# talmolab/VNL-Brax-Imitation

Hardware: AMD Instinct MI355X
Metric: env-steps/sec (whole node), rodent imitation, num_envs=4096/GPU (higher is better)
Workload: dtype f32; 1 GPU; rodent imitation rollout, single groom clip, 4096 envs/GPU: intention-policy forward (HIP) -> RodentTracking.step (5 substeps, CG 6/6) -> auto-reset on -> Transition logging (unroll 20, the 20 steps replayed as one captured hipGraph); envs_per_gpu=4096, clips=1, parallelism=env-sharded x1, no data-path collective

## Files before the change

__graft_entry__.py:

```python
from __future__ import annotations

import os
import sys

ROOT = os.path.dirname(os.path.abspath(__file__))
if ROOT not in sys.path:
    sys.path.insert(0, ROOT)


def build() -> None:
    import vnl_brax_imitation_amd
    from vnl_brax_imitation_amd.csrc import build as hip_build

    from concurrent.futures import ThreadPoolExecutor

    with ThreadPoolExecutor(8) as pool:
        futs = {v: pool.submit(hip_build.build, variant=v)
                for v in ("product", "spill", "noblk", "nospec", "tail", "plain", "vmemplain", "ldsplain")}
        paths = {v: f.result() for v, f in futs.items()}
    path = paths["product"]
    assert all(os.path.exists(p_) for p_ in paths.values()), paths
    from oracle import oracle as _oracle

    _oracle.build()
    from vnl_brax_imitation_amd import _lib

    _lib.load_library(path)
    print(f"[build] {path} ok; oracle ok")


def smoke() -> None:
    import numpy as np
    import torch

    sys.path.insert(0, os.path.join(ROOT, "tests"))
    import helpers as H
    from vnl_brax_imitation_amd.envs.rodent import RodentTracking

    assert torch.cuda.is_available(), "smoke() needs a HIP device"
    B = 256
    env = RodentTracking(H.reference_clip(), num_envs=B, device="cuda:0", **H.env_kwargs())
    rng = np.random.default_rng(0)
    sf = rng.integers(0, 235, B).astype(np.int32)
    noise = (1e-3 * rng.standard_normal((B, 74))).astype(np.float32)
    st = env.reset(start_frame=torch.from_numpy(sf), noise=torch.from_numpy(noise))
    act = np.clip(0.3 * rng.standard_normal((B, 30)), -1, 1).astype(np.float32)
    o = H.make_oracle(env, "f64")
    ost = o.env_reset(sf, noise)
    e_reset = H.scaled_err(st.pipeline_state.qacc_warmstart.cpu().numpy(), ost["qacc_warmstart"])
    e_obs = H.scaled_err(st.obs.cpu().numpy(), ost["obs"])
    import parity as P

    o32 = H.make_oracle(env, "f32")
    st, err, dev, rep, ost = P.control_step_follow(env, o, o32, sf, noise, act)
    torch.cuda.synchronize()
    print(f"[smoke] reset qacc err {e_reset:.2e}, obs err {e_obs:.2e}; control step vs oracle (following the product's "
          f"solver decisions): qvel err max {err['qvel'].max():.2e} median {np.median(err['qvel']):.2e}, qpos max "
          f"{err['qpos'].max():.2e}; reward {st.reward.mean().item():.5f} vs {ost['reward'].mean():.5f}")
    w = int(np.argmax(err["qvel"]))
    print(f"[smoke] worst env {w}: product vs float64 oracle {err['qvel'][w]:.2e}, float32 oracle vs float64 oracle "
          f"{dev['qvel'][w]:.2e} on the same env (bound: max(1e-5, {P.K_SENS} x that))")
    cp, co = P.compliance(err), P.compliance(dev)
    print(f"[smoke] envs within 1e-5 after ONE CONTROL STEP ({B} envs): product qpos {cp['qpos']:.3f} qvel {cp['qvel']:.3f} | "
          f"float32 oracle qpos {co['qpos']:.3f} qvel {co['qvel']:.3f}")
    env1 = RodentTracking(H.reference_clip(), num_envs=B, device="cuda:0", **{**H.env_kwargs(), "n_frames": 1})
    o1, o1_32 = H.make_oracle(env1, "f64"), H.make_oracle(env1, "f32")
    _, err1, dev1, rep1, _ = P.control_step_follow(env1, o1, o1_32, sf, noise, act)
    cp1, co1 = P.compliance(err1), P.compliance(dev1)
    print(f"[smoke] envs within 1e-5 after ONE SUBSTEP: product qpos {cp1['qpos']:.3f} qvel {cp1['qvel']:.3f} | float32 oracle "
          f"qpos {co1['qpos']:.3f} qvel {co1['qvel']:.3f}; followed decisions: {P.assert_legitimate(rep1)}")
    for f, idx in P.bound_violations(err1, dev1).items():
        assert len(idx) == 0, (f, idx[:8], err1[f][idx[:8]], dev1[f][idx[:8]])
    assert e_reset < 1e-4 and e_obs < 1e-5, (e_reset, e_obs)
    P.check_control_step(err, dev, rep)
    assert np.abs(st.reward.cpu().numpy() - ost["reward"]).max() < 2e-4
    assert np.array_equal(st.done.cpu().numpy(), ost["done"].astype(np.float32))
    assert torch.isfinite(st.obs).all()


if __name__ == "__main__":
    build()
    if "--smoke" in sys.argv:
        smoke()
```

vnl-brax-imitation_amd/csrc/build.py:

```python
from __future__ import annotations

import os
import subprocess
import sys

HERE = os.path.dirname(os.path.abspath(__file__))
SOURCES = ["vnl_lib.hip", "vnl_policy.hip", "vnl_ppo.hip", "vnl_domain.hip"]
DEPS = SOURCES + ["vnl_env_kernels.h", "vnl_body.h", "vnl_types.h", "vnl_philox.h", "vnl_policy_train.h", "../../include/vnl.h"]
OUT = os.path.join(HERE, "libvnl.so")

VARIANTS = {
    "product": ("libvnl.so", ["-DVNL_KERNEL_ATTR=__attribute__((amdgpu_waves_per_eu(2,2)))"]),
    "prof": ("libvnl_prof.so", ["-DVNL_PROFILE", "-DVNL_KERNEL_ATTR=__attribute__((amdgpu_waves_per_eu(2,2)))"]),
    "knobs": ("libvnl_knobs.so", ["-DVNL_STAGE_KNOBS", "-DVNL_KERNEL_ATTR=__attribute__((amdgpu_waves_per_eu(2,2)))"]),
    "spill": ("libvnl_spill.so", ["-DVNL_KERNEL_ATTR=__attribute__((amdgpu_waves_per_eu(4,4)))"]),
    "noblk": ("libvnl_noblk.so", ["-DVNL_NO_BLK", "-DVNL_KERNEL_ATTR=__attribute__((amdgpu_waves_per_eu(2,2)))"]),
    "tail": ("libvnl_tail.so", ["-DVNL_SOLVER_TAIL", "-DVNL_KERNEL_ATTR=__attribute__((amdgpu_waves_per_eu(2,2)))"]),
    "plain": ("libvnl_plain.so", ["-DVNL_SOLVER_PLAIN", "-DVNL_KERNEL_ATTR=__attribute__((amdgpu_waves_per_eu(2,2)))"]),
    "vmemplain": ("libvnl_vmemplain.so", ["-DVNL_VMEM_PLAIN", "-DVNL_KERNEL_ATTR=__attribute__((amdgpu_waves_per_eu(2,2)))"]),
    "ldsplain": ("libvnl_ldsplain.so", ["-DVNL_LDS_PLAIN", "-DVNL_KERNEL_ATTR=__attribute__((amdgpu_waves_per_eu(2,2)))"]),
    "nospec": ("libvnl_nospec.so", ["-DVNL_NO_SPEC", "-DVNL_KERNEL_ATTR=__attribute__((amdgpu_waves_per_eu(2,2)))"]),
}
ENV_KERNELS = ("vnl_step_kernel", "vnl_reset_kernel", "vnl_reset_done_kernel")


def resource_usage(stderr_text: str) -> dict:
    out, name = {}, None
    for line in stderr_text.splitlines():
        if "Function Name:" in line:
            name = line.split("Function Name:")[1].split()[0]
            out[name] = {}
        elif name and "remark:" in line:
            body = line.split("remark:")[1].split("[-Rpass")[0].strip()
            key, _, val = body.rpartition(":")
            try:
                out[name][key.strip()] = int(val.strip())
            except ValueError:
                pass
    return out


def build(force: bool = False, verbose: bool = False, profile: bool = False, knobs: bool = False,
          variant: str | None = None) -> str:
    variant = variant or ("prof" if profile else ("knobs" if knobs else "product"))
    fname, defs = VARIANTS[variant]
    out = os.path.join(HERE, fname)
    deps = [os.path.join(HERE, d) for d in DEPS] + [os.path.abspath(__file__)]
    newest = max(os.path.getmtime(d) for d in deps)
    if not force and os.path.exists(out) and os.path.getmtime(out) >= newest:
        return out
    hipcc = os.environ.get("HIPCC", "/opt/rocm/bin/hipcc")
    objdir = os.path.join(HERE, "_obj", variant)
    os.makedirs(objdir, exist_ok=True)
    flags = ["-Rpass-analysis=kernel-resource-usage", "--offload-arch=gfx950", "-O3", "-fno-slp-vectorize", "-std=c++17", "-fPIC"] + \
        defs + os.environ.get("VNL_HIPCC_EXTRA", "").split()
    stamp = " ".join(flags)
    headers = [d for d in deps if not d.endswith(".hip")]
    SRC_DEPS = {"vnl_lib.hip": headers, "vnl_policy.hip": [h for h in headers if h.endswith("vnl.h")] + [os.path.join(HERE, "vnl_policy_train.h"), os.path.join(HERE, "vnl_philox.h")],
                "vnl_ppo.hip": [h for h in headers if h.endswith("vnl.h")] + [os.path.join(HERE, "vnl_policy_train.h")]}
    objs, remarks = [], ""
    for src in SOURCES:
        obj = os.path.join(objdir, src + ".o")
        rem = obj + ".remarks.txt"
        srcdeps = [os.path.join(HERE, src)] + [h for h in SRC_DEPS.get(src, headers) if os.path.exists(h)]
        fresh = (not force and os.path.exists(obj) and os.path.exists(rem) and
                 os.path.getmtime(obj) >= max(os.path.getmtime(d) for d in srcdeps) and
                 open(rem).readline().rstrip("\n") == stamp)
        if not fresh:
            cmd = [hipcc] + flags + ["-c", os.path.join(HERE, src), "-o", obj]
            if verbose:
                print(" ".join(cmd), file=sys.stderr)
            r = subprocess.run(cmd, stderr=subprocess.PIPE, text=True)
            if verbose or r.returncode:
                sys.stderr.write(r.stderr)
            if r.returncode:
                raise subprocess.CalledProcessError(r.returncode, cmd)
            with open(rem, "w") as f:
                f.write(stamp + "\n" + r.stderr)
        objs.append(obj)
        remarks += open(rem).read().split("\n", 1)[1]
    cmd = [hipcc, "--offload-arch=gfx950", "-shared", "-fPIC", "-o", out] + objs
    r = subprocess.run(cmd, stderr=subprocess.PIPE, text=True)
    if r.returncode:
        sys.stderr.write(r.stderr)
        raise subprocess.CalledProcessError(r.returncode, cmd)

    class _R:
        stderr = remarks
    r = _R()
    usage = resource_usage(r.stderr)
    seen = {k: [u for n, u in usage.items() if k in n] for k in ENV_KERNELS}
    missing = [k for k, v in seen.items() if not v or "Occupancy [waves/SIMD]" not in v[0]]
    if missing:
        os.remove(out)
        raise RuntimeError(f"no resource-usage remark for {missing}: cannot check the register budget of this build")
    if variant == "product":
        for k, u in ((k, u) for k, v in seen.items() for u in v):
            if u.get("ScratchSize [bytes/lane]", 0) > 64 or u["Occupancy [waves/SIMD]"] < 2:
                if os.environ.get("VNL_ALLOW_SPILL") != "1":
                    os.remove(out)
                    raise RuntimeError(
                        f"{k}: {u.get('VGPRs')} VGPRs, {u.get('ScratchSize [bytes/lane]')} B scratch per lane, "
                        f"{u['Occupancy [waves/SIMD]']} waves/SIMD -- below the two waves per SIMD without spilling that the "
                        "published numbers were measured with.  Results do not depend on spilling (tests/test_gpu_spill.py); "
                        "this gate keeps a performance regression from shipping silently: set VNL_ALLOW_SPILL=1 to build anyway")
                sys.stderr.write(f"[build] WARNING (performance): {k} uses {u.get('VGPRs')} VGPRs, "
                                 f"{u.get('ScratchSize [bytes/lane]')} B scratch per lane, "
                                 f"{u['Occupancy [waves/SIMD]']} waves/SIMD: below the two waves per SIMD without "
                                 "spilling that the published numbers were measured with\n")
    with open(os.path.join(HERE, fname + ".resources.txt"), "w") as f:
        for n, u in usage.items():
            f.write(n + " " + " ".join(f"{a}={b}" for a, b in sorted(u.items())) + "\n")
    return out


if __name__ == "__main__":
    v = next((k for k in VARIANTS if "--" + k in sys.argv), None)
    if "--profile" in sys.argv:
        v = "prof"
    print(build(force="--force" in sys.argv, verbose=True, variant=v))
```

vnl-brax-imitation_amd/csrc/vnl_policy.hip:

```cpp
#include <hip/hip_runtime.h>
#include <math.h>
#include <stdint.h>
#include <stdio.h>

#include "../../include/vnl.h"
#include "vnl_philox.h"
#include "vnl_policy_train.h"

#define PT 16
#define PTHREADS 1024
#define PNT ((int)blockDim.x)
#define LN_EPS 1e-6f

typedef float v4f __attribute__((ext_vector_type(4)));


__device__ __forceinline__ int dense_col_groups(int N) {
  int G = (N + 63) >> 6, Gp = 1;
  while (Gp < G && Gp < PNT / 64) Gp <<= 1;
  return Gp;
}

template <bool VEC>
__device__ __forceinline__ void dense_tile_t(const float* X, int ldx, int K, const float* __restrict__ params, int w_off,
                                             int b_off, int N, float* Y, int ldy, bool relu, float* P, int split,
                                             int w2_off, int b2_off) {
  const float* __restrict__ bias = params + b_off;
  const float* __restrict__ bias2 = params + b2_off;
  const int tid = threadIdx.x, lane = tid & 63, wave = tid >> 6;
  const int j = lane & 15, kq = lane >> 4;
  const int G = (N + 63) >> 6, Gp = dense_col_groups(N), S = (PNT / 64) / Gp;
  const int g0 = wave & (Gp - 1), s = wave / Gp;
  const int N4 = (N + 3) & ~3;
  const int T = (K + 3) >> 2, Ts = (T + S - 1) / S;
  const int t0 = s * Ts, t1 = min(T, t0 + Ts);
  const float* xr = X + j * ldx + kq;
  float bias_r[4];
#pragma unroll
  for (int q = 0; q < 4; q++) {
    const int e = tid + q * PNT;
    const int c = e % N;
    bias_r[q] = e < PT * N ? (c < split ? bias[c] : bias2[c - split]) : 0.f;
  }
  const int ldw = split < N ? split : N;
  for (int g = g0; g < G; g += Gp) {
    const int c0 = g * 64 + 4 * j;
    auto load_b = [&](int step) -> v4f {
      const int k = 4 * step + kq;
      const float* w = params + (c0 < split ? w_off : w2_off - split) + (size_t)((step < t1 && k < K) ? k : 0) * ldw;
      v4f b;
      if (VEC) {
        b = *(const v4f*)(w + (c0 < N ? c0 : 0));
      } else {
#pragma unroll
        for (int t = 0; t < 4; t++) b[t] = w[c0 + t < N ? c0 + t : 0];
      }
      return b;
    };
    v4f acc[4];
#pragma unroll
    for (int t = 0; t < 4; t++) acc[t] = v4f{0.f, 0.f, 0.f, 0.f};
    auto mma4 = [&](const v4f (&b)[4], int t) {
      float a[4];
#pragma unroll
      for (int u = 0; u < 4; u++) {
        const int step = t + u;
        const bool ok = step < t1 && 4 * step + kq < K;
        float v = xr[ok ? 4 * step : 0];
        a[u] = ok ? v : 0.f;
      }
#pragma unroll
      for (int u = 0; u < 4; u++)
#pragma unroll
        for (int tt = 0; tt < 4; tt++) acc[tt] = __builtin_amdgcn_mfma_f32_16x16x4f32(a[u], b[u][tt], acc[tt], 0, 0, 0);
    };
    v4f b0[4], b1[4];
    if (t0 < t1) {
#pragma unroll
      for (int u = 0; u < 4; u++) b0[u] = load_b(t0 + u);
    }
    for (int t = t0; t < t1; t += 8) {
      const bool more1 = t + 4 < t1, more0 = t + 8 < t1;
      if (more1) {
#pragma unroll
        for (int u = 0; u < 4; u++) b1[u] = load_b(t + 4 + u);
      }
      __builtin_amdgcn_sched_barrier(0);
      mma4(b0, t);
      __builtin_amdgcn_sched_barrier(0);
      if (more0) {
#pragma unroll
        for (int u = 0; u < 4; u++) b0[u] = load_b(t + 8 + u);
      }
      __builtin_amdgcn_sched_barrier(0);
      if (more1) mma4(b1, t + 4);
      __builtin_amdgcn_sched_barrier(0);
    }
    if (c0 < N4) {
#pragma unroll
      for (int i = 0; i < 4; i++)
        *(v4f*)(P + (size_t)(s * PT + kq * 4 + i) * N4 + c0) = v4f{acc[0][i], acc[1][i], acc[2][i], acc[3][i]};
    }
  }
  __syncthreads();
  auto finish = [&](int e, float v) {
    const int r = e / N, c = e - r * N;
    for (int ss = 0; ss < S; ss++) v += P[(size_t)(ss * PT + r) * N4 + c];
    Y[r * ldy + c] = relu ? fmaxf(v, 0.f) : v;
  };
#pragma unroll
  for (int q = 0; q < 4; q++) {
    const int e = tid + q * PNT;
    if (e < PT * N) finish(e, bias_r[q]);
  }
  for (int e = tid + 4 * PNT; e < PT * N; e += PNT) finish(e, e % N < split ? bias[e % N] : bias2[e % N - split]);
  __syncthreads();
}

__device__ __forceinline__ void dense_tile(const float* X, int ldx, int K, const float* __restrict__ params, int w_off,
                                           int b_off, int N, float* Y, int ldy, bool relu, float* P, int split = 1 << 30,
                                           int w2_off = 0, int b2_off = 0) {
  const int ldw = split < N ? split : N;
  if ((ldw & 3) == 0 && ((uintptr_t)params & 15) == 0 && (w_off & 3) == 0 && (w2_off & 3) == 0)
    dense_tile_t<true>(X, ldx, K, params, w_off, b_off, N, Y, ldy, relu, P, split, w2_off, b2_off);
  else
    dense_tile_t<false>(X, ldx, K, params, w_off, b_off, N, Y, ldy, relu, P, split, w2_off, b2_off);
}

__device__ __forceinline__ void store_tile(const float* src, int ld, int nrow, int width, float* __restrict__ dst, int e0) {
  for (int i = threadIdx.x; i < nrow * width; i += PNT) {
    const int r = i / width, c = i - r * width;
    dst[(size_t)(e0 + r) * width + c] = src[r * ld + c];
  }
}

template <bool TRAIN>
__device__ __forceinline__ void layer_norm_rows(float* Y, int ldy, int N, const float* __restrict__ g,
                                                const float* __restrict__ be, float* __restrict__ stats = nullptr, int e0 = 0,
                                                int nrow = 0) {
  const int lane = threadIdx.x & 63, wave = threadIdx.x >> 6;
  const int RPW = PT / (PNT / 64);
  float gr[4], br[4];
#pragma unroll
  for (int q = 0; q < 4; q++) {
    const int c = lane + 64 * q;
    gr[q] = c < N ? g[c] : 0.f, br[q] = c < N ? be[c] : 0.f;
  }
  for (int r = wave * RPW; r < wave * RPW + RPW; r++) {
    float* y = Y + r * ldy;
    float s = 0.f, ss = 0.f;
    for (int c = lane; c < N; c += 64) {
      float v = y[c];
      s += v, ss += v * v;
    }
    for (int o = 32; o > 0; o >>= 1) s += __shfl_xor(s, o), ss += __shfl_xor(ss, o);
    float mean = s / (float)N;
    float var = fmaxf(ss / (float)N - mean * mean, 0.f);
    if (TRAIN) {
      float q = 0.f;
      for (int c = lane; c < N; c += 64) {
        const float d = y[c] - mean;
        q += d * d;
      }
      for (int o = 32; o > 0; o >>= 1) q += __shfl_xor(q, o);
      var = q / (float)N;
    }
    float inv = rsqrtf(var + LN_EPS);
    if (TRAIN && lane == 0 && r < nrow) stats[2 * (size_t)(e0 + r)] = mean, stats[2 * (size_t)(e0 + r) + 1] = inv;
#pragma unroll
    for (int q = 0; q < 4; q++) {
      const int c = lane + 64 * q;
      if (c < N) y[c] = (y[c] - mean) * inv * gr[q] + br[q];
    }
    for (int c = lane + 256; c < N; c += 64) y[c] = (y[c] - mean) * inv * g[c] + be[c];
  }
}

__device__ __forceinline__ void load_tile(const float* __restrict__ src, int nrow, int width, float* dst, int ld,
                                          const float* __restrict__ mean, const float* __restrict__ stdv) {
  const int tid = threadIdx.x, n = nrow * width;
  auto put = [&](int i, float v) {
    const int r = i / width, c = i - r * width;
    if (mean) v = (v - mean[c]) / stdv[c];
    dst[r * ld + c] = v;
  };
  int done = 0;
  if (((uintptr_t)src & 15) == 0) {
    const v4f* s4 = (const v4f*)src;
    const int n4 = n >> 2;
    for (int base = 0; base < n4; base += 4 * PNT) {
      v4f v[4];
#pragma unroll
      for (int u = 0; u < 4; u++) {
        const int i = base + u * PNT + tid;
        v[u] = s4[i < n4 ? i : 0];
      }
#pragma unroll
      for (int u = 0; u < 4; u++) {
        const int i = base + u * PNT + tid;
        if (i < n4) {
#pragma unroll
          for (int q = 0; q < 4; q++) put(4 * i + q, v[u][q]);
        }
      }
    }
    done = n4 << 2;
  }
  for (int i = done + tid; i < n; i += PNT) put(i, src[i]);
  for (int i = n + tid; i < PT * width; i += PNT) {
    const int r = i / width, c = i - r * width;
    dst[r * ld + c] = 0.f;
  }
}

#ifdef VNL_PROFILE
__device__ long long g_policy_stamps[32];
#define POL_STAMP(i)                                                               \
  do {                                                                             \
    if (blockIdx.x == 0 && threadIdx.x == 0) g_policy_stamps[i] = wall_clock64(); \
  } while (0)
extern "C" int vnl_policy_profile_stamps(long long* out) {
  return hipMemcpyFromSymbol(out, HIP_SYMBOL(g_policy_stamps), sizeof(long long) * 32) == hipSuccess ? 0 : -1;
}
#else
#define POL_STAMP(i)
#endif

__device__ __forceinline__ float softplusf(float x) { return x > 20.f ? x : log1pf(expf(x)); }

struct PolicyNoiseDev {
  uint32_t key0, key1;
  const int64_t* step_base;
  int64_t step_offset;
  uint32_t env0;
  float *eps_latent_out, *eps_action_out, *rand_action_out;
};


__device__ __forceinline__ void draw_normal_tile(const PolicyNoiseDev& nz, int64_t step, uint32_t stream, int e0, int nrow, int n,
                                                 float* dst, float* __restrict__ rec) {
  const int nb = (n + 3) >> 2;
  const uint32_t c2 = (uint32_t)step, c3 = ((uint32_t)(step >> 32) << 2) | stream;
  for (int i = threadIdx.x; i < nrow * nb; i += PNT) {
    const int r = i / nb, b = i - r * nb;
    uint32_t x[4];
    philox4x32_10((uint32_t)b, nz.env0 + (uint32_t)(e0 + r), c2, c3, nz.key0, nz.key1, x);
    float v[4];
    box_muller(x[0], x[1], v[0], v[1]);
    box_muller(x[2], x[3], v[2], v[3]);
    *(v4f*)(dst + (r * nb + b) * 4) = v4f{v[0], v[1], v[2], v[3]};
    if (rec) {
#pragma unroll
      for (int q = 0; q < 4; q++)
        if (4 * b + q < n) rec[(size_t)(e0 + r) * n + 4 * b + q] = v[q];
    }
  }
}

template <int MODE>
__global__ void __launch_bounds__(PTHREADS) vnl_policy_kernel_t(PolicyDev p, const float* __restrict__ params,
                                                              const float* __restrict__ obs_mean,
                                                              const float* __restrict__ obs_std,
                                                              const float* __restrict__ traj, const float* __restrict__ obs,
                                                              const float* __restrict__ eps_latent,
                                                              const float* __restrict__ eps_action, int batch,
                                                              int deterministic, float* __restrict__ action,
                                                              float* __restrict__ raw_action, float* __restrict__ log_prob,
                                                              float* __restrict__ logits, float* __restrict__ lat_mean,
                                                              float* __restrict__ lat_logvar,
                                                              const float* __restrict__ rand_action,
                                                              float* __restrict__ rand_log_prob, PolicyTrainOut t,
                                                              PolicyNoiseDev nz) {
  extern __shared__ __align__(16) float lds[];
  float* A = lds;
  float* B = lds + PT * p.ldA;
  float* P = B + PT * p.ldB;
  const int e0 = blockIdx.x * PT, tid = threadIdx.x;
  const int nrow = min(PT, batch - e0);

  constexpr bool TRAIN = MODE == 1 || MODE == 2;
  constexpr bool DRAW = MODE == 3;
  const int64_t step = DRAW ? *nz.step_base + nz.step_offset : 0;
  if (TRAIN) __builtin_amdgcn_s_setprio(3);
  POL_STAMP(0);
  float *X = A, *Y = B;
  int ldx = p.ldA, ldy = p.ldB, K = p.traj_size;
  if (MODE == 2) {
    load_tile(t.encH[0] + (size_t)e0 * p.enc[0], nrow, p.enc[0], Y, ldy, nullptr, nullptr);
  } else {
    load_tile(traj + (size_t)e0 * p.traj_size, nrow, p.traj_size, A, p.ldA, nullptr, nullptr);
  }
  __syncthreads();
  POL_STAMP(1);
  for (int l = 0; l < p.n_enc; l++) {
    if (!(MODE == 2 && l == 0)) {
      dense_tile(X, ldx, K, params, p.enc_w[l], p.enc_b[l], p.enc[l], Y, ldy, true, P);
      POL_STAMP(2 + 2 * l);
      if (TRAIN) {
        store_tile(Y, ldy, nrow, p.enc[l], t.encH[l], e0);
        __syncthreads();
      }
    }
    layer_norm_rows<TRAIN>(Y, ldy, p.enc[l], params + p.enc_g[l], params + p.enc_be[l], t.encS[l], e0, nrow);
    __syncthreads();
    if (TRAIN) store_tile(Y, ldy, nrow, p.enc[l], t.encY[l], e0);
    POL_STAMP(3 + 2 * l);
    float* t = X;
    X = Y, Y = t;
    int tl = ldx;
    ldx = ldy, ldy = tl;
    K = p.enc[l];
  }
  if ((p.latent & 63) == 0) {
    dense_tile(X, ldx, K, params, p.mean_w, p.mean_b, 2 * p.latent, Y, ldy, false, P, p.latent, p.lv_w, p.lv_b);
  } else {
    dense_tile(X, ldx, K, params, p.mean_w, p.mean_b, p.latent, Y, ldy, false, P);
    dense_tile(X, ldx, K, params, p.lv_w, p.lv_b, p.latent, Y + p.latent, ldy, false, P);
  }
  POL_STAMP(10);
  if (TRAIN) store_tile(Y, ldy, nrow, 2 * p.latent, t.ml, e0);
  const int lat4 = (p.latent + 3) & ~3;
  if (DRAW) {
    draw_normal_tile(nz, step, 0u, e0, nrow, p.latent, P, nz.eps_latent_out);
    __syncthreads();
  }
  for (int i = tid; i < PT * p.latent; i += PNT) {
    int r = i / p.latent, c = i - r * p.latent;
    float mu = Y[r * ldy + c], lv = Y[r * ldy + p.latent + c];
    float z = 0.f;
    if (r < nrow) {
      size_t g = (size_t)(e0 + r) * p.latent + c;
      lat_mean[g] = mu, lat_logvar[g] = lv;
      z = mu + (DRAW ? P[r * lat4 + c] : eps_latent[g]) * expf(0.5f * lv);
    }
    X[r * ldx + c] = z;
  }
  load_tile(obs + (size_t)e0 * p.obs_size, nrow, p.obs_size, X + p.latent, ldx, obs_mean, obs_std);
  __syncthreads();
  if (TRAIN) store_tile(X, ldx, nrow, p.latent + p.obs_size, t.D0, e0);
  POL_STAMP(11);
  K = p.latent + p.obs_size;
  for (int l = 0; l < p.n_dec; l++) {
    bool last = l == p.n_dec - 1;
    dense_tile(X, ldx, K, params, p.dec_w[l], p.dec_b[l], p.dec[l], Y, ldy, !last, P);
    POL_STAMP(12 + 2 * l);
    if (!last) {
      if (TRAIN) {
        store_tile(Y, ldy, nrow, p.dec[l], t.decH[l], e0);
        __syncthreads();
      }
      layer_norm_rows<TRAIN>(Y, ldy, p.dec[l], params + p.dec_g[l], params + p.dec_be[l], t.decS[l], e0, nrow);
      __syncthreads();
      if (TRAIN) store_tile(Y, ldy, nrow, p.dec[l], t.decY[l], e0);
    }
    float* t = X;
    X = Y, Y = t;
    int tl = ldx;
    ldx = ldy, ldy = tl;
    K = p.dec[l];
  }
  POL_STAMP(20);
  const int na = p.act_size;
  for (int i = tid; i < PT * 2 * na; i += PNT) {
    int r = i / (2 * na), c = i - r * 2 * na;
    if (r < nrow) logits[(size_t)(e0 + r) * 2 * na + c] = X[r * ldx + c];
  }
  if (TRAIN) return;
  float* lp = Y;
  const bool has_rand = DRAW ? rand_log_prob != nullptr : rand_action != nullptr;
  const int act4 = (na + 3) & ~3;
  if (DRAW && !deterministic) {
    draw_normal_tile(nz, step, 1u, e0, nrow, na, P, nz.eps_action_out);
    if (has_rand && tid < (act4 >> 2)) {
      uint32_t x[4];
      philox4x32_10((uint32_t)tid, 0xFFFFFFFFu, (uint32_t)step, ((uint32_t)(step >> 32) << 2) | 2u, nz.key0, nz.key1, x);
#pragma unroll
      for (int q = 0; q < 4; q++) {
        const float v = (float)((int)(2u * (x[q] >> 8) + 1u) - (1 << 24)) * 0x1p-24f;
        P[PT * act4 + 4 * tid + q] = v;
        if (blockIdx.x == 0 && nz.rand_action_out && 4 * tid + q < na) nz.rand_action_out[4 * tid + q] = v;
      }
    }
    __syncthreads();
  }
  for (int i = tid; i < PT * na; i += PNT) {
    int r = i / na, c = i - r * na;
    float term = 0.f;
    if (r < nrow) {
      size_t g = (size_t)(e0 + r) * na + c;
      float loc = X[r * ldx + c];
      if (deterministic) {
        action[g] = tanhf(loc);
      } else {
        float scale = softplusf(X[r * ldx + na + c]) + 0.001f;
        float eps = DRAW ? P[r * act4 + c] : eps_action[g];
        float raw = loc + scale * eps;
        raw_action[g] = raw, action[g] = tanhf(raw);
        term = -0.5f * eps * eps - 0.9189385332046727f - logf(scale) - 2.f * (0.6931471805599453f - raw - softplusf(-2.f * raw));
        if (has_rand) {
          float x = DRAW ? P[PT * act4 + c] : rand_action[c], z = (x - loc) / scale;
          lp[r * ldy + na + c] = -0.5f * z * z - 0.9189385332046727f - logf(scale) - 2.f * (0.6931471805599453f - x - softplusf(-2.f * x));
        }
      }
    }
    lp[r * ldy + c] = term;
  }
  __syncthreads();
  if (!deterministic && tid < nrow) {
    float s = 0.f;
    for (int c = 0; c < na; c++) s += lp[tid * ldy + c];
    log_prob[e0 + tid] = s;
    if (has_rand) {
      float s2 = 0.f;
      for (int c = 0; c < na; c++) s2 += lp[tid * ldy + na + c];
      rand_log_prob[e0 + tid] = s2;
    }
  }
  POL_STAMP(21);
}

void vnl_set_error_(const char* msg);
static int pfail(int code, const char* msg) {
  vnl_set_error_(msg);
  return code;
}

struct vnl_policy {
  PolicyDev d;
  int device, max_batch;
  int64_t nparams;
  size_t lds_bytes;
  PolicyDev d2;
  size_t lds_bytes2;
  int threads2;
};

int vnl_policy_set_threads2_(vnl_policy* p, int threads) {
  if (!p || (threads != 256 && threads != 512 && threads != 1024)) return VNL_ERR_ARG;
  const PolicyDev& d = p->d;
  int pw2 = 0;
  bool ok2 = true;
  auto upd2 = [&](int n) {
    int G = (n + 63) / 64, Gp = 1;
    while (Gp < G && Gp < threads / 64) Gp <<= 1;
    if (G > Gp) ok2 = false;
    int w = (threads / 64 / Gp) * ((n + 3) & ~3);
    pw2 = w > pw2 ? w : pw2;
  };
  for (int l = 0; l < d.n_enc; l++) upd2(d.enc[l]);
  for (int l = 0; l < d.n_dec; l++) upd2(d.dec[l]);
  upd2(d.latent), upd2(2 * d.latent);
  if (!ok2) return VNL_ERR_UNSUPPORTED;
  p->threads2 = threads;
  p->lds_bytes2 = (size_t)PT * (2 * d.ldB + pw2) * sizeof(float);
  return VNL_OK;
}

extern "C" int vnl_policy_create(const vnl_policy_spec* s, int32_t max_batch, int32_t device, vnl_policy** out) {
  if (!s || !out) return pfail(VNL_ERR_ARG, "vnl_policy_create: null argument");
  if (s->num_encoder_layers < 1 || s->num_encoder_layers > 8 || s->num_decoder_layers < 1 || s->num_decoder_layers > 8)
    return pfail(VNL_ERR_UNSUPPORTED, "1..8 encoder and decoder layers supported");
  if (s->decoder_layers[s->num_decoder_layers - 1] != 2 * s->action_size)
    return pfail(VNL_ERR_ARG, "last decoder layer must be 2 * action_size (NormalTanh parameters)");
  int ndev = 0;
  if (hipGetDeviceCount(&ndev) != hipSuccess || ndev <= 0) return pfail(VNL_ERR_NO_DEVICE, "no HIP device (no CPU fallback)");
  if (device < 0 || device >= ndev) return pfail(VNL_ERR_ARG, "device ordinal out of range");
  vnl_policy* p = new vnl_policy();
  PolicyDev& d = p->d;
  d.traj_size = s->traj_size, d.obs_size = s->obs_size, d.act_size = s->action_size, d.latent = s->latent_size;
  d.n_enc = s->num_encoder_layers, d.n_dec = s->num_decoder_layers;
  int off = 0, fan = d.traj_size;
  for (int l = 0; l < d.n_enc; l++) {
    int h = d.enc[l] = s->encoder_layers[l];
    d.enc_w[l] = off, off += fan * h;
    d.enc_b[l] = off, off += h;
    d.enc_g[l] = off, off += h;
    d.enc_be[l] = off, off += h;
    fan = h;
  }
  d.mean_w = off, off += fan * d.latent;
  d.mean_b = off, off += d.latent;
  d.lv_w = off, off += fan * d.latent;
  d.lv_b = off, off += d.latent;
  fan = d.latent + d.obs_size;
  for (int l = 0; l < d.n_dec; l++) {
    int h = d.dec[l] = s->decoder_layers[l];
    d.dec_w[l] = off, off += fan * h;
    d.dec_b[l] = off, off += h;
    if (l != d.n_dec - 1) {
      d.dec_g[l] = off, off += h;
      d.dec_be[l] = off, off += h;
    }
    fan = h;
  }
  p->nparams = off;
  int wa = d.traj_size, wb = 2 * d.latent;
  bool toB = true;
  auto put = [&](int w) {
    if (toB) wb = w > wb ? w : wb; else wa = w > wa ? w : wa;
    toB = !toB;
  };
  for (int l = 0; l < d.n_enc; l++) put(d.enc[l]);
  {
    int w_heads = 2 * d.latent, w_in = d.latent + d.obs_size;
    if (toB) wb = w_heads > wb ? w_heads : wb; else wa = w_heads > wa ? w_heads : wa;
    if (toB) wa = w_in > wa ? w_in : wa; else wb = w_in > wb ? w_in : wb;
  }
  for (int l = 0; l < d.n_dec; l++) put(d.dec[l]);
  wa = wa > wb ? wa : wb;
  int wide = 0;
  for (int l = 0; l < d.n_enc; l++) wide = d.enc[l] > wide ? d.enc[l] : wide;
  for (int l = 0; l < d.n_dec; l++) wide = d.dec[l] > wide ? d.dec[l] : wide;
  wide = wide > d.latent + d.obs_size ? wide : d.latent + d.obs_size;
  wide = wide > 2 * d.latent ? wide : 2 * d.latent;
  int la = d.traj_size > wide ? d.traj_size : wide;
  auto pad = [](int w) { return ((w + 29) / 32) * 32 + 2; };
  d.ldA = pad(la), d.ldB = pad(wide);
  int pw = 0;
  auto part = [&](int n) {
    int G = (n + 63) / 64, Gp = 1;
    while (Gp < G && Gp < PTHREADS / 64) Gp <<= 1;
    int w = (PTHREADS / 64 / Gp) * ((n + 3) & ~3);
    if (G > Gp) w = -1;
    return w;
  };
  bool too_wide = false;
  auto upd = [&](int n) {
    int w = part(n);
    if (w < 0) too_wide = true;
    pw = w > pw ? w : pw;
  };
  for (int l = 0; l < d.n_enc; l++) upd(d.enc[l]);
  for (int l = 0; l < d.n_dec; l++) upd(d.dec[l]);
  upd(d.latent), upd(2 * d.latent);
  if (too_wide) {
    delete p;
    return pfail(VNL_ERR_UNSUPPORTED, "layers wider than 1024 are not supported by the fused policy kernel");
  }
  p->lds_bytes = (size_t)PT * (d.ldA + d.ldB + pw) * sizeof(float);
  if (p->lds_bytes > 160 * 1024 - 512) {
    delete p;
    return pfail(VNL_ERR_UNSUPPORTED, "network too wide for the 16-env LDS tile");
  }
  p->d2 = d, p->d2.ldA = d.ldB;
  (void)vnl_policy_set_threads2_(p, PTHREADS);
  p->device = device, p->max_batch = max_batch;
  if (p->lds_bytes > 64 * 1024) {
    hipError_t e = hipFuncSetAttribute((const void*)vnl_policy_kernel_t<0>, hipFuncAttributeMaxDynamicSharedMemorySize,
                                       (int)p->lds_bytes);
    if (e == hipSuccess)
      e = hipFuncSetAttribute((const void*)vnl_policy_kernel_t<3>, hipFuncAttributeMaxDynamicSharedMemorySize, (int)p->lds_bytes);
    if (e == hipSuccess)
      e = hipFuncSetAttribute((const void*)vnl_policy_kernel_t<1>, hipFuncAttributeMaxDynamicSharedMemorySize, (int)p->lds_bytes);
    if (e == hipSuccess)
      e = hipFuncSetAttribute((const void*)vnl_policy_kernel_t<2>, hipFuncAttributeMaxDynamicSharedMemorySize, (int)p->lds_bytes2);
    if (e != hipSuccess) {
      delete p;
      return pfail(VNL_ERR_HIP, hipGetErrorString(e));
    }
  }
  *out = p;
  return VNL_OK;
}

extern "C" void vnl_policy_destroy(vnl_policy* p) { delete p; }
extern "C" int64_t vnl_policy_num_params(const vnl_policy* p) { return p ? p->nparams : -1; }

extern "C" int vnl_policy_forward(vnl_policy* p, const float* params, const float* obs_mean, const float* obs_std,
                                  const float* traj, const float* obs, const float* eps_latent, const float* eps_action,
                                  int32_t batch, int32_t deterministic, float* action, float* raw_action, float* log_prob,
                                  float* logits, float* latent_mean, float* latent_logvar, const float* rand_action,
// ... 70 lines not shown
```

Baseline: 2.713 million env-steps/s.

## Prefetch next layer weights, layernorm params and obs across policy MLP layers

Restructures the policy forward kernel so that each dense layer issues the first weight loads of the following layer (and the layernorm gamma/beta) before its reduction barrier. It also prefetches observations, latent/action noise and rand_action into registers ahead of use. Bias/row index arithmetic replaces per-element divides, and the log-prob sums are split across two thread groups. This aims to hide global-memory latency between the serial MLP layers, at the cost of more register pressure. A plain build variant keeps the old path for comparison.

New measurement: 2.713 million env-steps/s. No clear change (-0.0%).

```diff
diff --git a/__graft_entry__.py b/__graft_entry__.py
--- a/__graft_entry__.py
+++ b/__graft_entry__.py
@@ -14,9 +14,9 @@
 
     from concurrent.futures import ThreadPoolExecutor
 
-    with ThreadPoolExecutor(8) as pool:
+    with ThreadPoolExecutor(9) as pool:
         futs = {v: pool.submit(hip_build.build, variant=v)
-                for v in ("product", "spill", "noblk", "nospec", "tail", "plain", "vmemplain", "ldsplain")}
+                for v in ("product", "spill", "noblk", "nospec", "tail", "plain", "vmemplain", "ldsplain", "polplain")}
         paths = {v: f.result() for v, f in futs.items()}
     path = paths["product"]
     assert all(os.path.exists(p_) for p_ in paths.values()), paths
diff --git a/vnl-brax-imitation_amd/csrc/build.py b/vnl-brax-imitation_amd/csrc/build.py
--- a/vnl-brax-imitation_amd/csrc/build.py
+++ b/vnl-brax-imitation_amd/csrc/build.py
@@ -19,6 +19,7 @@
     "plain": ("libvnl_plain.so", ["-DVNL_SOLVER_PLAIN", "-DVNL_KERNEL_ATTR=__attribute__((amdgpu_waves_per_eu(2,2)))"]),
     "vmemplain": ("libvnl_vmemplain.so", ["-DVNL_VMEM_PLAIN", "-DVNL_KERNEL_ATTR=__attribute__((amdgpu_waves_per_eu(2,2)))"]),
     "ldsplain": ("libvnl_ldsplain.so", ["-DVNL_LDS_PLAIN", "-DVNL_KERNEL_ATTR=__attribute__((amdgpu_waves_per_eu(2,2)))"]),
+    "polplain": ("libvnl_polplain.so", ["-DVNL_POLICY_PLAIN", "-DVNL_KERNEL_ATTR=__attribute__((amdgpu_waves_per_eu(2,2)))"]),
     "nospec": ("libvnl_nospec.so", ["-DVNL_NO_SPEC", "-DVNL_KERNEL_ATTR=__attribute__((amdgpu_waves_per_eu(2,2)))"]),
 }
 ENV_KERNELS = ("vnl_step_kernel", "vnl_reset_kernel", "vnl_reset_done_kernel")
diff --git a/vnl-brax-imitation_amd/csrc/vnl_policy.hip b/vnl-brax-imitation_amd/csrc/vnl_policy.hip
--- a/vnl-brax-imitation_amd/csrc/vnl_policy.hip
+++ b/vnl-brax-imitation_amd/csrc/vnl_policy.hip
@@ -15,116 +15,199 @@
 typedef float v4f __attribute__((ext_vector_type(4)));
 
 
+#ifdef VNL_POLICY_PLAIN
+#define POL_AHEAD false
+#else
+#define POL_AHEAD true
+#endif
+template <bool V>
+struct PolBool {
+  static constexpr bool value = V;
+};
+
 __device__ __forceinline__ int dense_col_groups(int N) {
   int G = (N + 63) >> 6, Gp = 1;
   while (Gp < G && Gp < PNT / 64) Gp <<= 1;
   return Gp;
 }
 
+struct DenseSlice {
+  int K, N, split, w_off, w2_off;
+  int G, S;
+  int g, s, t0, t1;
+};
+
+__device__ __forceinline__ DenseSlice dense_slice(int K, int N, int w_off, int split = 1 << 30, int w2_off = 0) {
+  DenseSlice d;
+  d.K = K, d.N = N, d.split = split, d.w_off = w_off, d.w2_off = w2_off;
+  const int wave = __builtin_amdgcn_readfirstlane(threadIdx.x >> 6), Gp = dense_col_groups(N);
+  d.G = (N + 63) >> 6, d.S = (PNT / 64) / Gp;
+  d.g = wave & (Gp - 1), d.s = wave / Gp;
+  const int T = (K + 3) >> 2, Ts = (T + d.S - 1) / d.S;
+  d.t0 = d.s * Ts;
+  d.t1 = d.g < d.G ? min(T, d.t0 + Ts) : d.t0;
+  return d;
+}
+
 template <bool VEC>
-__device__ __forceinline__ void dense_tile_t(const float* X, int ldx, int K, const float* __restrict__ params, int w_off,
-                                             int b_off, int N, float* Y, int ldy, bool relu, float* P, int split,
-                                             int w2_off, int b2_off) {
+__device__ __forceinline__ v4f dense_load_b(const DenseSlice& d, const float* __restrict__ params, int step) {
+  const int lane = threadIdx.x & 63, c0 = d.g * 64 + 4 * (lane & 15), k = 4 * step + (lane >> 4);
+  const int ldw = d.split < d.N ? d.split : d.N;
+  const float* w = params + (c0 < d.split ? d.w_off : d.w2_off - d.split) + (size_t)((step < d.t1 && k < d.K) ? k : 0) * ldw;
+  v4f b;
+  if (VEC) {
+    b = *(const v4f*)(w + (c0 < d.N ? c0 : 0));
+  } else {
+#pragma unroll
+    for (int t = 0; t < 4; t++) b[t] = w[c0 + t < d.N ? c0 + t : 0];
+  }
+  return b;
+}
+
+struct WeightSets {
+  v4f b0[4], b1[4];
+};
+
+template <bool VEC>
+__device__ __forceinline__ void dense_prefetch(const DenseSlice& d, const float* __restrict__ params, WeightSets& w) {
+  if (d.t0 < d.t1) {
+#pragma unroll
+    for (int u = 0; u < 4; u++) w.b0[u] = dense_load_b<VEC>(d, params, d.t0 + u);
+  }
+  if (VEC && d.t0 + 4 < d.t1) {
+#pragma unroll
+    for (int u = 0; u < 4; u++) w.b1[u] = dense_load_b<VEC>(d, params, d.t0 + 4 + u);
+  }
+  __builtin_amdgcn_sched_barrier(0);
+}
+
+struct LnRegs {
+  float g[4], b[4];
+};
+__device__ __forceinline__ void ln_request(int N, const float* __restrict__ g, const float* __restrict__ be, LnRegs& r) {
+  const int lane = threadIdx.x & 63;
+#pragma unroll
+  for (int q = 0; q < 4; q++) {
+    const int c = lane + 64 * q;
+    r.g[q] = c < N ? g[c] : 0.f, r.b[q] = c < N ? be[c] : 0.f;
+  }
+}
+
+template <bool VEC, bool CHAIN>
+__device__ __forceinline__ void dense_tile_t(const float* X, int ldx, const float* __restrict__ params, const DenseSlice& d,
+                                             int b_off, int b2_off, float* Y, int ldy, bool relu, float* P, WeightSets& chained,
+                                             bool has_next, const DenseSlice& nx, bool want_ln, LnRegs& ln,
+                                             const float* __restrict__ ln_g, const float* __restrict__ ln_b) {
+  WeightSets own;
+  WeightSets& w = CHAIN ? chained : own;
   const float* __restrict__ bias = params + b_off;
   const float* __restrict__ bias2 = params + b2_off;
-  const int tid = threadIdx.x, lane = tid & 63, wave = tid >> 6;
+  const int tid = threadIdx.x, lane = tid & 63;
   const int j = lane & 15, kq = lane >> 4;
-  const int G = (N + 63) >> 6, Gp = dense_col_groups(N), S = (PNT / 64) / Gp;
-  const int g0 = wave & (Gp - 1), s = wave / Gp;
+  const int K = d.K, N = d.N, S = d.S, split = d.split, t0 = d.t0, t1 = d.t1;
   const int N4 = (N + 3) & ~3;
-  const int T = (K + 3) >> 2, Ts = (T + S - 1) / S;
-  const int t0 = s * Ts, t1 = min(T, t0 + Ts);
   const float* xr = X + j * ldx + kq;
+  const int dq = PNT / N, dc = PNT - dq * N;
+  const int r0 = tid / N, c0e = tid - r0 * N;
+  auto advance = [&](int& r, int& c) {
+    r += dq, c += dc;
+    if (c >= N) c -= N, r++;
+  };
   float bias_r[4];
-#pragma unroll
-  for (int q = 0; q < 4; q++) {
-    const int e = tid + q * PNT;
-    const int c = e % N;
-    bias_r[q] = e < PT * N ? (c < split ? bias[c] : bias2[c - split]) : 0.f;
-  }
-  const int ldw = split < N ? split : N;
-  for (int g = g0; g < G; g += Gp) {
-    const int c0 = g * 64 + 4 * j;
-    auto load_b = [&](int step) -> v4f {
-      const int k = 4 * step + kq;
-      const float* w = params + (c0 < split ? w_off : w2_off - split) + (size_t)((step < t1 && k < K) ? k : 0) * ldw;
-      v4f b;
-      if (VEC) {
-        b = *(const v4f*)(w + (c0 < N ? c0 : 0));
-      } else {
-#pragma unroll
-        for (int t = 0; t < 4; t++) b[t] = w[c0 + t < N ? c0 + t : 0];
-      }
-      return b;
-    };
-    v4f acc[4];
-#pragma unroll
-    for (int t = 0; t < 4; t++) acc[t] = v4f{0.f, 0.f, 0.f, 0.f};
-    auto mma4 = [&](const v4f (&b)[4], int t) {
-      float a[4];
-#pragma unroll
-      for (int u = 0; u < 4; u++) {
-        const int step = t + u;
-        const bool ok = step < t1 && 4 * step + kq < K;
-        float v = xr[ok ? 4 * step : 0];
-        a[u] = ok ? v : 0.f;
-      }
-#pragma unroll
-      for (int u = 0; u < 4; u++)
-#pragma unroll
-        for (int tt = 0; tt < 4; tt++) acc[tt] = __builtin_amdgcn_mfma_f32_16x16x4f32(a[u], b[u][tt], acc[tt], 0, 0, 0);
-    };
-    v4f b0[4], b1[4];
-    if (t0 < t1) {
-#pragma unroll
-      for (int u = 0; u < 4; u++) b0[u] = load_b(t0 + u);
-    }
-    for (int t = t0; t < t1; t += 8) {
-      const bool more1 = t + 4 < t1, more0 = t + 8 < t1;
-      if (more1) {
-#pragma unroll
-        for (int u = 0; u < 4; u++) b1[u] = load_b(t + 4 + u);
-      }
-      __builtin_amdgcn_sched_barrier(0);
-      mma4(b0, t);
-      __builtin_amdgcn_sched_barrier(0);
-      if (more0) {
-#pragma unroll
-        for (int u = 0; u < 4; u++) b0[u] = load_b(t + 8 + u);
-      }
-      __builtin_amdgcn_sched_barrier(0);
-      if (more1) mma4(b1, t + 4);
-      __builtin_amdgcn_sched_barrier(0);
-    }
-    if (c0 < N4) {
-#pragma unroll
-      for (int i = 0; i < 4; i++)
-        *(v4f*)(P + (size_t)(s * PT + kq * 4 + i) * N4 + c0) = v4f{acc[0][i], acc[1][i], acc[2][i], acc[3][i]};
-    }
-  }
+  {
+    int r = r0, c = c0e;
+#pragma unroll
+    for (int q = 0; q < 4; q++) {
+      const int e = tid + q * PNT;
+      bias_r[q] = e < PT * N ? (c < split ? bias[c] : bias2[c - split]) : 0.f;
+      advance(r, c);
+    }
+  }
+  if (!CHAIN) dense_prefetch<VEC>(d, params, w);
+  v4f acc[4];
+#pragma unroll
+  for (int t = 0; t < 4; t++) acc[t] = v4f{0.f, 0.f, 0.f, 0.f};
+  auto mma4 = [&](const v4f (&b)[4], int t) {
+    float a[4];
+#pragma unroll
+    for (int u = 0; u < 4; u++) {
+      const int step = t + u;
+      const bool ok = step < t1 && 4 * step + kq < K;
+      float v = xr[ok ? 4 * step : 0];
+      a[u] = ok ? v : 0.f;
+    }
+#pragma unroll
+    for (int u = 0; u < 4; u++)
+#pragma unroll
+      for (int tt = 0; tt < 4; tt++) acc[tt] = __builtin_amdgcn_mfma_f32_16x16x4f32(a[u], b[u][tt], acc[tt], 0, 0, 0);
+  };
+  for (int t = t0; t < t1; t += 8) {
+    const bool more1 = t + 4 < t1, more0 = t + 8 < t1, more2 = t + 12 < t1;
+    if (!VEC && more1) {
+#pragma unroll
+      for (int u = 0; u < 4; u++) w.b1[u] = dense_load_b<VEC>(d, params, t + 4 + u);
+    }
+    __builtin_amdgcn_sched_barrier(0);
+    mma4(w.b0, t);
+    __builtin_amdgcn_sched_barrier(0);
+    if (more0) {
+#pragma unroll
+      for (int u = 0; u < 4; u++) w.b0[u] = dense_load_b<VEC>(d, params, t + 8 + u);
+    }
+    __builtin_amdgcn_sched_barrier(0);
+    if (more1) mma4(w.b1, t + 4);
+    __builtin_amdgcn_sched_barrier(0);
+    if (VEC && more2) {
+#pragma unroll
+      for (int u = 0; u < 4; u++) w.b1[u] = dense_load_b<VEC>(d, params, t + 12 + u);
+    }
+  }
+  if (CHAIN) {
+#pragma unroll
+    for (int q = 0; q < 4; q++) asm volatile("" : "+v"(bias_r[q]));
+    if (has_next) dense_prefetch<VEC>(nx, params, w);
+  }
+  const int c0 = d.g * 64 + 4 * j;
+  if (d.g < d.G && c0 < N4) {
+#pragma unroll
+    for (int i = 0; i < 4; i++)
+      *(v4f*)(P + (size_t)(d.s * PT + kq * 4 + i) * N4 + c0) = v4f{acc[0][i], acc[1][i], acc[2][i], acc[3][i]};
+  }
+  if (want_ln) ln_request(N, ln_g, ln_b, ln);
   __syncthreads();
-  auto finish = [&](int e, float v) {
-    const int r = e / N, c = e - r * N;
+  auto finish = [&](int r, int c, float v) {
     for (int ss = 0; ss < S; ss++) v += P[(size_t)(ss * PT + r) * N4 + c];
     Y[r * ldy + c] = relu ? fmaxf(v, 0.f) : v;
   };
-#pragma unroll
-  for (int q = 0; q < 4; q++) {
-    const int e = tid + q * PNT;
-    if (e < PT * N) finish(e, bias_r[q]);
-  }
-  for (int e = tid + 4 * PNT; e < PT * N; e += PNT) finish(e, e % N < split ? bias[e % N] : bias2[e % N - split]);
+  {
+    int r = r0, c = c0e;
+#pragma unroll
+    for (int q = 0; q < 4; q++) {
+      const int e = tid + q * PNT;
+      if (e < PT * N) finish(r, c, bias_r[q]);
+      advance(r, c);
+    }
+  }
+  for (int e = tid + 4 * PNT; e < PT * N; e += PNT) finish(e / N, e % N, e % N < split ? bias[e % N] : bias2[e % N - split]);
   __syncthreads();
 }
 
-__device__ __forceinline__ void dense_tile(const float* X, int ldx, int K, const float* __restrict__ params, int w_off,
-                                           int b_off, int N, float* Y, int ldy, bool relu, float* P, int split = 1 << 30,
-                                           int w2_off = 0, int b2_off = 0) {
-  const int ldw = split < N ? split : N;
-  if ((ldw & 3) == 0 && ((uintptr_t)params & 15) == 0 && (w_off & 3) == 0 && (w2_off & 3) == 0)
-    dense_tile_t<true>(X, ldx, K, params, w_off, b_off, N, Y, ldy, relu, P, split, w2_off, b2_off);
+__device__ __forceinline__ bool dense_vec_ok(const float* params, int w_off, int w2_off, int ldw) {
+  return (ldw & 3) == 0 && ((uintptr_t)params & 15) == 0 && (w_off & 3) == 0 && (w2_off & 3) == 0;
+}
+template <bool CHAIN>
+__device__ __forceinline__ void dense_tile(const float* X, int ldx, const float* __restrict__ params, const DenseSlice& d,
+                                           int b_off, int b2_off, float* Y, int ldy, bool relu, float* P, WeightSets& w,
+                                           bool has_next, const DenseSlice& nx, bool want_ln, LnRegs& ln,
+                                           const float* __restrict__ ln_g, const float* __restrict__ ln_b) {
+  if (CHAIN) {
+    dense_tile_t<true, true>(X, ldx, params, d, b_off, b2_off, Y, ldy, relu, P, w, has_next, nx, want_ln, ln, ln_g, ln_b);
+    return;
+  }
+  if (dense_vec_ok(params, d.w_off, d.w2_off, d.split < d.N ? d.split : d.N))
+    dense_tile_t<true, false>(X, ldx, params, d, b_off, b2_off, Y, ldy, relu, P, w, has_next, nx, want_ln, ln, ln_g, ln_b);
   else
-    dense_tile_t<false>(X, ldx, K, params, w_off, b_off, N, Y, ldy, relu, P, split, w2_off, b2_off);
+    dense_tile_t<false, false>(X, ldx, params, d, b_off, b2_off, Y, ldy, relu, P, w, has_next, nx, want_ln, ln, ln_g, ln_b);
 }
 
 __device__ __forceinline__ void store_tile(const float* src, int ld, int nrow, int width, float* __restrict__ dst, int e0) {
@@ -136,16 +219,11 @@
 
 template <bool TRAIN>
 __device__ __forceinline__ void layer_norm_rows(float* Y, int ldy, int N, const float* __restrict__ g,
-                                                const float* __restrict__ be, float* __restrict__ stats = nullptr, int e0 = 0,
-                                                int nrow = 0) {
-  const int lane = threadIdx.x & 63, wave = threadIdx.x >> 6;
+                                                const float* __restrict__ be, const LnRegs& pre,
+                                                float* __restrict__ stats = nullptr, int e0 = 0, int nrow = 0) {
+  const int lane = threadIdx.x & 63, wave = __builtin_amdgcn_readfirstlane(threadIdx.x >> 6);
   const int RPW = PT / (PNT / 64);
-  float gr[4], br[4];
-#pragma unroll
-  for (int q = 0; q < 4; q++) {
-    const int c = lane + 64 * q;
-    gr[q] = c < N ? g[c] : 0.f, br[q] = c < N ? be[c] : 0.f;
-  }
+  const float(&gr)[4] = pre.g, (&br)[4] = pre.b;
   for (int r = wave * RPW; r < wave * RPW + RPW; r++) {
     float* y = Y + r * ldy;
     float s = 0.f, ss = 0.f;
@@ -199,8 +277,14 @@
       for (int u = 0; u < 4; u++) {
         const int i = base + u * PNT + tid;
         if (i < n4) {
-#pragma unroll
-          for (int q = 0; q < 4; q++) put(4 * i + q, v[u][q]);
+          int r = 4 * i / width, c = 4 * i - r * width;
+#pragma unroll
+          for (int q = 0; q < 4; q++) {
+            float x = v[u][q];
+            if (mean) x = (x - mean[c]) / stdv[c];
+            dst[r * ld + c] = x;
+            if (++c == width) c = 0, r++;
+          }
         }
       }
     }
@@ -210,6 +294,39 @@
   for (int i = n + tid; i < PT * width; i += PNT) {
     const int r = i / width, c = i - r * width;
     dst[r * ld + c] = 0.f;
+  }
+}
+
+struct ObsRegs {
+  v4f v, m, sd;
+};
+__device__ __forceinline__ bool obs_ahead_ok(const float* src, int width, const float* mean, const float* stdv) {
+  return POL_AHEAD && (width & 3) == 0 && PT * width <= 4 * PNT &&
+         ((((uintptr_t)src | (uintptr_t)mean | (uintptr_t)stdv) & 15) == 0);
+}
+__device__ __forceinline__ void obs_request(const float* __restrict__ src, int nrow, int width, ObsRegs& o) {
+  const int i = threadIdx.x, n4 = (nrow * width) >> 2;
+  if (i < n4) o.v = ((const v4f*)src)[i];
+}
+__device__ __forceinline__ void obs_request_stats(int nrow, int width, const float* __restrict__ mean,
+                                                  const float* __restrict__ stdv, ObsRegs& o) {
+  const int i = threadIdx.x, n4 = (nrow * width) >> 2;
+  const int r = 4 * i / width, c = 4 * i - r * width;
+  if (mean && i < n4) o.m = *(const v4f*)(mean + c), o.sd = *(const v4f*)(stdv + c);
+}
+__device__ __forceinline__ void obs_put(const ObsRegs& o, int nrow, int width, bool normalise, float* dst, int ld) {
+  const int i = threadIdx.x, n4 = (nrow * width) >> 2;
+  if (4 * i < PT * width) {
+    const int r = 4 * i / width, c = 4 * i - r * width;
+#pragma unroll
+    for (int q = 0; q < 4; q++) {
+      float x = 0.f;
+      if (i < n4) {
+        x = o.v[q];
+        if (normalise) x = (x - o.m[q]) / o.sd[q];
+      }
+      dst[r * ld + c + q] = x;
+    }
   }
 }
 
@@ -280,11 +397,33 @@
 
   constexpr bool TRAIN = MODE == 1 || MODE == 2;
   constexpr bool DRAW = MODE == 3;
+  constexpr bool LN_AHEAD = POL_AHEAD && MODE != 2;
   const int64_t step = DRAW ? *nz.step_base + nz.step_offset : 0;
   if (TRAIN) __builtin_amdgcn_s_setprio(3);
+  bool vec_all = POL_AHEAD;
+  {
+    auto ok = [&](int w_off, int ldw) { vec_all = vec_all && dense_vec_ok(params, w_off, 0, ldw); };
+    for (int l = 0; l < p.n_enc; l++) ok(p.enc_w[l], p.enc[l]);
+    ok(p.mean_w, p.latent), ok(p.lv_w, p.latent);
+    for (int l = 0; l < p.n_dec; l++) ok(p.dec_w[l], p.dec[l]);
+  }
+  auto body = [&](auto chain_c) {
+  constexpr bool CHAIN = decltype(chain_c)::value;
   POL_STAMP(0);
   float *X = A, *Y = B;
-  int ldx = p.ldA, ldy = p.ldB, K = p.traj_size;
+  int ldx = p.ldA, ldy = p.ldB;
+  const bool one_head = (p.latent & 63) == 0;
+  const int k_heads = p.enc[p.n_enc - 1];
+  auto enc_slice = [&](int l) { return dense_slice(l ? p.enc[l - 1] : p.traj_size, p.enc[l], p.enc_w[l]); };
+  auto head_slice = [&](int h) {
+    return one_head ? dense_slice(k_heads, 2 * p.latent, p.mean_w, p.latent, p.lv_w)
+                    : dense_slice(k_heads, p.latent, h ? p.lv_w : p.mean_w);
+  };
+  auto dec_slice = [&](int l) { return dense_slice(l ? p.dec[l - 1] : p.latent + p.obs_size, p.dec[l], p.dec_w[l]); };
+  WeightSets w;
+  LnRegs ln;
+  DenseSlice cur = MODE == 2 ? (p.n_enc > 1 ? enc_slice(1) : head_slice(0)) : enc_slice(0), nx = cur;
+  if (CHAIN) dense_prefetch<true>(cur, params, w);
   if (MODE == 2) {
     load_tile(t.encH[0] + (size_t)e0 * p.enc[0], nrow, p.enc[0], Y, ldy, nullptr, nullptr);
   } else {
@@ -293,15 +432,20 @@
   __syncthreads();
   POL_STAMP(1);
   for (int l = 0; l < p.n_enc; l++) {
-    if (!(MODE == 2 && l == 0)) {
-      dense_tile(X, ldx, K, params, p.enc_w[l], p.enc_b[l], p.enc[l], Y, ldy, true, P);
+    const float *ln_g = params + p.enc_g[l], *ln_b = params + p.enc_be[l];
+    const bool dense_here = !(MODE == 2 && l == 0);
+    if (dense_here) {
+      nx = l + 1 < p.n_enc ? enc_slice(l + 1) : head_slice(0);
+      dense_tile<CHAIN>(X, ldx, params, cur, p.enc_b[l], 0, Y, ldy, true, P, w, true, nx, LN_AHEAD, ln, ln_g, ln_b);
+      cur = nx;
       POL_STAMP(2 + 2 * l);
       if (TRAIN) {
         store_tile(Y, ldy, nrow, p.enc[l], t.encH[l], e0);
         __syncthreads();
       }
     }
-    layer_norm_rows<TRAIN>(Y, ldy, p.enc[l], params + p.enc_g[l], params + p.enc_be[l], t.encS[l], e0, nrow);
+    if (!LN_AHEAD || !dense_here) ln_request(p.enc[l], ln_g, ln_b, ln);
+    layer_norm_rows<TRAIN>(Y, ldy, p.enc[l], ln_g, ln_b, ln, t.encS[l], e0, nrow);
     __syncthreads();
     if (TRAIN) store_tile(Y, ldy, nrow, p.enc[l], t.encY[l], e0);
     POL_STAMP(3 + 2 * l);
@@ -309,15 +453,27 @@
     X = Y, Y = t;
     int tl = ldx;
     ldx = ldy, ldy = tl;
-    K = p.enc[l];
-  }
-  if ((p.latent & 63) == 0) {
-    dense_tile(X, ldx, K, params, p.mean_w, p.mean_b, 2 * p.latent, Y, ldy, false, P, p.latent, p.lv_w, p.lv_b);
+  }
+  const float* obs_src = obs + (size_t)e0 * p.obs_size;
+  const bool obs_ahead = obs_ahead_ok(obs_src, p.obs_size, obs_mean, obs_std);
+  ObsRegs obs_r;
+  float eps_l0 = 0.f;
+  if (obs_ahead && !TRAIN) obs_request(obs_src, nrow, p.obs_size, obs_r);
+  if (POL_AHEAD && !DRAW && tid < nrow * p.latent) eps_l0 = eps_latent[(size_t)e0 * p.latent + tid];
+  if (one_head) {
+    nx = dec_slice(0);
+    dense_tile<CHAIN>(X, ldx, params, cur, p.mean_b, p.lv_b, Y, ldy, false, P, w, true, nx, false, ln, params, params);
+    cur = nx;
   } else {
-    dense_tile(X, ldx, K, params, p.mean_w, p.mean_b, p.latent, Y, ldy, false, P);
-    dense_tile(X, ldx, K, params, p.lv_w, p.lv_b, p.latent, Y + p.latent, ldy, false, P);
+    nx = head_slice(1);
+    dense_tile<CHAIN>(X, ldx, params, cur, p.mean_b, 0, Y, ldy, false, P, w, true, nx, false, ln, params, params);
+    cur = nx, nx = dec_slice(0);
+    dense_tile<CHAIN>(X, ldx, params, cur, p.lv_b, 0, Y + p.latent, ldy, false, P, w, true, nx, false, ln, params, params);
+    cur = nx;
   }
   POL_STAMP(10);
+  if (obs_ahead && TRAIN) obs_request(obs_src, nrow, p.obs_size, obs_r);
+  if (obs_ahead) obs_request_stats(nrow, p.obs_size, obs_mean, obs_std, obs_r);
   if (TRAIN) store_tile(Y, ldy, nrow, 2 * p.latent, t.ml, e0);
   const int lat4 = (p.latent + 3) & ~3;
   if (DRAW) {
@@ -331,25 +487,38 @@
     if (r < nrow) {
       size_t g = (size_t)(e0 + r) * p.latent + c;
       lat_mean[g] = mu, lat_logvar[g] = lv;
-      z = mu + (DRAW ? P[r * lat4 + c] : eps_latent[g]) * expf(0.5f * lv);
+      z = mu + (DRAW ? P[r * lat4 + c] : (POL_AHEAD && i == tid ? eps_l0 : eps_latent[g])) * expf(0.5f * lv);
     }
     X[r * ldx + c] = z;
   }
-  load_tile(obs + (size_t)e0 * p.obs_size, nrow, p.obs_size, X + p.latent, ldx, obs_mean, obs_std);
+  if (obs_ahead)
+    obs_put(obs_r, nrow, p.obs_size, obs_mean != nullptr, X + p.latent, ldx);
+  else
+    load_tile(obs_src, nrow, p.obs_size, X + p.latent, ldx, obs_mean, obs_std);
   __syncthreads();
   if (TRAIN) store_tile(X, ldx, nrow, p.latent + p.obs_size, t.D0, e0);
   POL_STAMP(11);
-  K = p.latent + p.obs_size;
+  const int na = p.act_size;
+  const bool has_rand = DRAW ? rand_log_prob != nullptr : rand_action != nullptr;
+  float eps_a0 = 0.f, rand_a0 = 0.f;
   for (int l = 0; l < p.n_dec; l++) {
     bool last = l == p.n_dec - 1;
-    dense_tile(X, ldx, K, params, p.dec_w[l], p.dec_b[l], p.dec[l], Y, ldy, !last, P);
+    const float *ln_g = params + p.dec_g[last ? 0 : l], *ln_b = params + p.dec_be[last ? 0 : l];
+    if (POL_AHEAD && MODE == 0 && last && !deterministic && tid < nrow * na) {
+      eps_a0 = eps_action[(size_t)e0 * na + tid];
+      if (has_rand) rand_a0 = rand_action[tid % na];
+    }
+    nx = last ? cur : dec_slice(l + 1);
+    dense_tile<CHAIN>(X, ldx, params, cur, p.dec_b[l], 0, Y, ldy, !last, P, w, !last, nx, LN_AHEAD && !last, ln, ln_g, ln_b);
+    cur = nx;
     POL_STAMP(12 + 2 * l);
     if (!last) {
       if (TRAIN) {
         store_tile(Y, ldy, nrow, p.dec[l], t.decH[l], e0);
         __syncthreads();
       }
-      layer_norm_rows<TRAIN>(Y, ldy, p.dec[l], params + p.dec_g[l], params + p.dec_be[l], t.decS[l], e0, nrow);
+      if (!LN_AHEAD) ln_request(p.dec[l], ln_g, ln_b, ln);
+      layer_norm_rows<TRAIN>(Y, ldy, p.dec[l], ln_g, ln_b, ln, t.decS[l], e0, nrow);
       __syncthreads();
       if (TRAIN) store_tile(Y, ldy, nrow, p.dec[l], t.decY[l], e0);
     }
@@ -357,17 +526,14 @@
     X = Y, Y = t;
     int tl = ldx;
     ldx = ldy, ldy = tl;
-    K = p.dec[l];
   }
   POL_STAMP(20);
-  const int na = p.act_size;
   for (int i = tid; i < PT * 2 * na; i += PNT) {
     int r = i / (2 * na), c = i - r * 2 * na;
     if (r < nrow) logits[(size_t)(e0 + r) * 2 * na + c] = X[r * ldx + c];
   }
   if (TRAIN) return;
   float* lp = Y;
-  const bool has_rand = DRAW ? rand_log_prob != nullptr : rand_action != nullptr;
   const int act4 = (na + 3) & ~3;
   if (DRAW && !deterministic) {
     draw_normal_tile(nz, step, 1u, e0, nrow, na, P, nz.eps_action_out);
@@ -393,12 +559,13 @@
         action[g] = tanhf(loc);
       } else {
         float scale = softplusf(X[r * ldx + na + c]) + 0.001f;
-        float eps = DRAW ? P[r * act4 + c] : eps_action[g];
+        const bool first = POL_AHEAD && MODE == 0 && i == tid;
+        float eps = DRAW ? P[r * act4 + c] : (first ? eps_a0 : eps_action[g]);
         float raw = loc + scale * eps;
         raw_action[g] = raw, action[g] = tanhf(raw);
         term = -0.5f * eps * eps - 0.9189385332046727f - logf(scale) - 2.f * (0.6931471805599453f - raw - softplusf(-2.f * raw));
         if (has_rand) {
-          float x = DRAW ? P[PT * act4 + c] : rand_action[c], z = (x - loc) / scale;
+          float x = DRAW ? P[PT * act4 + c] : (first ? rand_a0 : rand_action[c]), z = (x - loc) / scale;
           lp[r * ldy + na + c] = -0.5f * z * z - 0.9189385332046727f - logf(scale) - 2.f * (0.6931471805599453f - x - softplusf(-2.f * x));
         }
       }
@@ -406,17 +573,26 @@
     lp[r * ldy + c] = term;
   }
   __syncthreads();
-  if (!deterministic && tid < nrow) {
+  const int sum_row = POL_AHEAD ? tid & (PT - 1) : tid, sum_of = POL_AHEAD ? tid >> 4 : 0;
+  if (!deterministic && sum_row < nrow && sum_of < (POL_AHEAD && has_rand ? 2 : 1)) {
     float s = 0.f;
-    for (int c = 0; c < na; c++) s += lp[tid * ldy + c];
-    log_prob[e0 + tid] = s;
-    if (has_rand) {
+    for (int c = 0; c < na; c++) s += lp[sum_row * ldy + sum_of * na + c];
+    (sum_of ? rand_log_prob : log_prob)[e0 + sum_row] = s;
+    if (!POL_AHEAD && has_rand) {
       float s2 = 0.f;
-      for (int c = 0; c < na; c++) s2 += lp[tid * ldy + na + c];
-      rand_log_prob[e0 + tid] = s2;
+      for (int c = 0; c < na; c++) s2 += lp[sum_row * ldy + na + c];
+      rand_log_prob[e0 + sum_row] = s2;
     }
   }
   POL_STAMP(21);
+  };
+  if constexpr (POL_AHEAD) {
+    if (vec_all) {
+      body(PolBool<true>{});
+      return;
+    }
+  }
+  body(PolBool<false>{});
 }
 
 void vnl_set_error_(const char* msg);
```
